# kkty/kmer-sets-compression

Hardware: AMD Instinct MI355X
Metric: Mk-mers/s processed in kmerset-multiple-compress; bytes/k-mer after SPSS (higher is better)
Workload: dtype u32

## Files before the change

include/kmersets_hip.h:

```cpp
#ifndef KMERSETS_HIP_H_
#define KMERSETS_HIP_H_

#include <stddef.h>
#include <stdint.h>

#ifdef __cplusplus
extern "C" {
#endif

#define KSH_OK 0
#define KSH_INVALID_ARGUMENT 3
#define KSH_FAILED_PRECONDITION 9
#define KSH_INTERNAL 13

typedef struct ksh_ctx ksh_ctx;

typedef struct ksh_geom {
  int32_t k;
  int32_t n_bucket_bits;
  int32_t key_bytes;
  int32_t reserved;
} ksh_geom;

typedef struct ksh_set_view {
// ... 105 lines not shown
  KSH_ROUTE_RC_256 = 1 << 3,
  KSH_ROUTE_RC_64 = 1 << 4,
  KSH_ROUTE_RC_BATCHED = 1 << 5,
  KSH_ROUTE_SCATTER_TWO_LEVEL = 1 << 6,
  KSH_ROUTE_FWD_STAGED = 1 << 7,
  KSH_ROUTE_RANK_ONE_LAUNCH = 1 << 8,
  KSH_ROUTE_HEADS_ONE_LAUNCH = 1 << 9,
  KSH_ROUTE_JUMP_TWO_LEVEL = 1 << 10,
  KSH_ROUTE_RANK_STAMPED = 1 << 11,
  KSH_ROUTE_EMIT_LOGS = 1 << 12,
  KSH_ROUTE_LONG_STRETCHES = 1 << 13,
  KSH_ROUTE_MATCH_MORE_ROUNDS = 1 << 14,
  KSH_ROUTE_FWD_TARGETS = 1 << 15,
  KSH_ROUTE_RC1_STREAMED = 1 << 16,
  KSH_ROUTE_RC_MARKS_GROUPS = 1 << 17,
  KSH_ROUTE_TGT_PARTS = 1 << 18
};
int ksh_spss_encode_routes(ksh_ctx* ctx, int64_t* routes);
int ksh_spss_encode_release(ksh_ctx* ctx);

int ksh_spss_cover_plan(ksh_ctx* ctx, const ksh_geom* g, const ksh_spss_view* unitigs, int canonical, int fast,
                        int64_t* n_strings, int64_t* n_bases);
int ksh_spss_cover_write(ksh_ctx* ctx, uint64_t* d_words, uint32_t* d_lens);
int ksh_spss_cover_stats(ksh_ctx* ctx, int64_t stats[4]);
int ksh_spss_cover_release(ksh_ctx* ctx);

typedef struct ksh_kss ksh_kss;
int ksh_kss_build(ksh_ctx* ctx, const ksh_geom* g, const ksh_spss_view* inputs, int32_t n_inputs,
                  const int32_t* bucket_ids, int32_t n_ids, int canonical, int32_t max_iterations,
                  ksh_kss** out);
typedef int (*ksh_allgather_i64)(void* user, const int64_t* send, int64_t count, int64_t* recv);
// ... 66 lines not shown
```

kmer-sets-compression_amd/csrc/ksh_decode.hip:

```cpp
#include "ksh_internal.h"
#include "ksh_kmer.h"

#include <algorithm>
#include <cstdlib>
#include <string>
#include <vector>

namespace ksh {

constexpr int kDecThreads = 1024;
constexpr int kMaxLdsBuckets = 16384;
constexpr int kSortLdsBytes = 63488;
constexpr int kMaxSubBits = 11;
constexpr int kSortThreads = 1024;

__global__ __launch_bounds__(256) void k_str_bases(const uint32_t* __restrict__ lens, int64_t n,
                                                    int k, int64_t* __restrict__ bases) {
  const int64_t i = int64_t(blockIdx.x) * blockDim.x + threadIdx.x;
  if (i < n) bases[i] = int64_t(lens[i]) + k;
}

__global__ __launch_bounds__(256) void k_mark_ends(const int64_t* __restrict__ str_start,
                                                    int64_t n_strings,
                                                    unsigned long long* __restrict__ end_bits) {
  const int64_t i = int64_t(blockIdx.x) * blockDim.x + threadIdx.x;
  if (i >= n_strings) return;
  const int64_t p = str_start[i + 1] - 1;
  atomicOr(&end_bits[p >> 6], 1ull << (p & 63));
}
// ... 236 lines not shown
#pragma unroll
  for (int j = 0; j < kDecL2Per; j++) {
    if (bin[j] == 0xFFFFFFFFu) continue;
    const uint32_t pos = s_lbase[bin[j]] + rank[j];
    s_key[pos] = mine[j];
    s_bin[pos] = uint16_t(bin[j]);
  }
  __syncthreads();
  const uint32_t staged = s_lbase[kBins - 1] + s_cnt[kBins - 1];
  for (uint32_t i = tid; i < staged; i += kDecL2Threads) {
    const uint32_t b = s_bin[i];
    keys[s_gbase[b] + (i - s_lbase[b])] = s_key[i];
  }
}

constexpr int kColTeams = 16;
__global__ __launch_bounds__(64 * kColTeams) void k_hist_columns(uint32_t* __restrict__ hist_matrix,
                                                                  int64_t n_groups, int n_buckets,
                                                                  int64_t* __restrict__ totals,
                                                                  unsigned long long* __restrict__ max_total) {
  __shared__ uint32_t team_total[kColTeams][64];
  const int lane = threadIdx.x & 63, team = threadIdx.x >> 6;
  const int b = blockIdx.x * 64 + lane;
  const int64_t per_team = (n_groups + kColTeams - 1) / kColTeams;
  const int64_t g0 = min(int64_t(team) * per_team, n_groups), g1 = min(g0 + per_team, n_groups);
  uint32_t run = 0;
  if (b < n_buckets)
    for (int64_t g = g0; g < g1; g++) run += hist_matrix[g * n_buckets + b];
  team_total[team][lane] = run;
  __syncthreads();
// ... 24 lines not shown
      if (lane == 0 && max_total) atomicMax(max_total, m);
    } else if (max_total) {
      atomicMax(max_total, m);
    }
  }
}

struct SortLds {
  uint32_t sub_cnt[(1 << kMaxSubBits) + 1];
  int wave_cnt[kSortThreads / 64];
  int wave_below[kSortThreads / 64];
  int overflow;
  int kept;
};

template <typename KeyT>
__device__ void block_sort_into_lds(const KeyT* __restrict__ src, int cnt, int eff_bits,
                                    KeyT* __restrict__ lds, SortLds* __restrict__ sh) {
  int bits = 0;
  while ((4 << bits) < cnt && bits < kMaxSubBits) bits++;
  if (bits > eff_bits) bits = eff_bits;
  const int n_sub = 1 << bits;
  const int shift = eff_bits - bits;
  for (int i = threadIdx.x; i <= n_sub; i += kSortThreads) sh->sub_cnt[i] = 0;
  if (threadIdx.x == 0) sh->overflow = 0;
  constexpr int kSortRegs = 8;
  const bool in_regs = cnt <= kSortRegs * kSortThreads;
  KeyT held[kSortRegs];
  if (in_regs) {
#pragma unroll
    for (int u = 0; u < kSortRegs; u++) {
      const int i = int(threadIdx.x) + u * kSortThreads;
      if (i < cnt) held[u] = src[i];
    }
  }
  __syncthreads();
  if (in_regs) {
#pragma unroll
    for (int u = 0; u < kSortRegs; u++)
      if (int(threadIdx.x) + u * kSortThreads < cnt)
        atomicAdd(&sh->sub_cnt[uint32_t(uint64_t(held[u]) >> shift) & uint32_t(n_sub - 1)], 1u);
  } else {
    for (int i = threadIdx.x; i < cnt; i += kSortThreads)
      atomicAdd(&sh->sub_cnt[uint32_t(uint64_t(src[i]) >> shift) & uint32_t(n_sub - 1)], 1u);
  }
  __syncthreads();
  {
    const int per = (n_sub + kSortThreads - 1) / kSortThreads;
    const int c0 = min(int(threadIdx.x) * per, n_sub), c1 = min(c0 + per, n_sub);
    int mine = 0;
    for (int i = c0; i < c1; i++) mine += int(sh->sub_cnt[i]);
    const int lane = threadIdx.x & 63, wave = threadIdx.x >> 6;
    int inc = mine;
#pragma unroll
    for (int d = 1; d < 64; d <<= 1) {
      const int o = __shfl_up(inc, d, 64);
      if (lane >= d) inc += o;
    }
    if (lane == 63) sh->wave_cnt[wave] = inc;
    __syncthreads();
    int run = inc - mine;
    for (int w = 0; w < wave; w++) run += sh->wave_cnt[w];
    for (int i = c0; i < c1; i++) {
      const int c = int(sh->sub_cnt[i]);
      sh->sub_cnt[i] = uint32_t(run);
      run += c;
    }
  }
  __syncthreads();
  if (in_regs) {
#pragma unroll
    for (int u = 0; u < kSortRegs; u++)
      if (int(threadIdx.x) + u * kSortThreads < cnt) {
        const uint32_t pos = atomicAdd(&sh->sub_cnt[uint32_t(uint64_t(held[u]) >> shift) & uint32_t(n_sub - 1)], 1u);
        lds[pos] = held[u];
      }
  } else {
    for (int i = threadIdx.x; i < cnt; i += kSortThreads) {
      const KeyT key = src[i];
      const uint32_t pos = atomicAdd(&sh->sub_cnt[uint32_t(uint64_t(key) >> shift) & uint32_t(n_sub - 1)], 1u);
      lds[pos] = key;
    }
  }
  __syncthreads();
  for (int b2 = threadIdx.x; b2 < n_sub; b2 += kSortThreads) {
    const int s0 = b2 ? int(sh->sub_cnt[b2 - 1]) : 0, s1 = int(sh->sub_cnt[b2]);
    if (s1 - s0 > 64) {
      sh->overflow = 1;
    } else {
      for (int i = s0 + 1; i < s1; i++) {
        const KeyT x = lds[i];
        int j = i - 1;
        while (j >= s0 && lds[j] > x) {
          lds[j + 1] = lds[j];
          j--;
        }
        lds[j + 1] = x;
      }
    }
  }
  __syncthreads();
  if (sh->overflow == 0) return;
  int padded = 1;
  while (padded < cnt) padded <<= 1;
  const int half = padded >> 1;
  for (int size = 2; size <= padded; size <<= 1) {
    const int hs = size >> 1;
    for (int p = threadIdx.x; p < half; p += kSortThreads) {
      const int block = p / hs, o = p - block * hs;
      const int i = block * size + o, j = block * size + size - 1 - o;
      if (j < cnt) {
        const KeyT x = lds[i], y = lds[j];
        if (x > y) {
          lds[i] = y;
          lds[j] = x;
        }
      }
    }
    __syncthreads();
    for (int stride = size >> 2; stride > 0; stride >>= 1) {
      for (int p = threadIdx.x; p < half; p += kSortThreads) {
        const int i = 2 * stride * (p / stride) + (p % stride), j = i + stride;
        if (j < cnt) {
          const KeyT x = lds[i], y = lds[j];
          if (x > y) {
            lds[i] = y;
            lds[j] = x;
          }
        }
      }
      __syncthreads();
    }
  }
}

template <typename KeyT>
__device__ int block_unique_write(const KeyT* __restrict__ lds, int cnt, KeyT* __restrict__ dst,
                                  SortLds* __restrict__ sh, int cutoff, int64_t* below) {
  const int per = (cnt + kSortThreads - 1) / kSortThreads;
  const int c0 = min(int(threadIdx.x) * per, cnt), c1 = min(c0 + per, cnt);
  int mine = 0, mine_below = 0;
  for (int i = c0; i < c1; i++) {
    if (i == 0 || lds[i] != lds[i - 1]) {
      bool keep = true;
      if (cutoff > 1) {
        int run = 1;
        while (run < cutoff && i + run < cnt && lds[i + run] == lds[i]) run++;
        keep = run >= cutoff;
      }
      mine += keep;
      mine_below += !keep;
    }
  }
  const int lane = threadIdx.x & 63, wave = threadIdx.x >> 6;
// ... 1 lines not shown
#pragma unroll
  for (int d = 1; d < 64; d <<= 1) {
    const int o = __shfl_up(inc, d, 64);
    if (lane >= d) inc += o;
  }
#pragma unroll
  for (int d = 32; d >= 1; d >>= 1) inc_below += __shfl_xor(inc_below, d, 64);
  __syncthreads();
  if (lane == 63) sh->wave_cnt[wave] = inc;
  if (lane == 0) sh->wave_below[wave] = inc_below;
  __syncthreads();
  int at = inc - mine;
  for (int w = 0; w < wave; w++) at += sh->wave_cnt[w];
  int total = 0;
#pragma unroll
  for (int w = 0; w < kSortThreads / 64; w++) total += sh->wave_cnt[w];
  if (threadIdx.x == 0 && below)
    for (int w = 0; w < kSortThreads / 64; w++) *below += sh->wave_below[w];
  if (total == cnt) {
    for (int i = threadIdx.x; i < cnt; i += kSortThreads) dst[i] = lds[i];
    __syncthreads();
    return total;
  }
  for (int i = c0; i < c1; i++) {
    if (i == 0 || lds[i] != lds[i - 1]) {
      bool keep = true;
      if (cutoff > 1) {
        int run = 1;
        while (run < cutoff && i + run < cnt && lds[i + run] == lds[i]) run++;
        keep = run >= cutoff;
      }
      if (keep) dst[at++] = lds[i];
    }
  }
  __syncthreads();
  return total;
}

template <typename KeyT>
__global__ __launch_bounds__(kSortThreads, 8) void k_bucket_sort(const int64_t* __restrict__ offsets,
                                                      KeyT* __restrict__ keys,
                                                      KeyT* __restrict__ scratch,
                                                      int64_t* __restrict__ uniq, int key_bits,
                                                      int cutoff, int64_t* __restrict__ below) {
  extern __shared__ unsigned char lds_raw[];
  __shared__ SortLds sh;
  __shared__ uint32_t part_end[(1 << kMaxSubBits) + 1];
  KeyT* lds = reinterpret_cast<KeyT*>(lds_raw);
  constexpr int kCap = kSortLdsBytes / int(sizeof(KeyT));
  const int64_t b = blockIdx.x;
  const int64_t lo = offsets[b], hi = offsets[b + 1];
  const int64_t cnt64 = hi - lo;
  if (cnt64 == 0) {
    if (threadIdx.x == 0) {
      uniq[b] = 0;
      if (below) below[b] = 0;
    }
    return;
  }
  KeyT* g = keys + lo;
  int64_t n_below = 0;
  if (cnt64 <= kCap) {
    block_sort_into_lds(g, int(cnt64), key_bits, lds, &sh);
    const int kept = block_unique_write(lds, int(cnt64), g, &sh, cutoff, &n_below);
    if (threadIdx.x == 0) {
      uniq[b] = kept;
      if (below) below[b] = n_below;
    }
    return;
  }
  KeyT* tmp = scratch + lo;
  int bits = 1;
  while ((cnt64 >> bits) > kCap / 4 && bits < kMaxSubBits) bits++;
  if (bits > key_bits) bits = key_bits;
  const int n_part = 1 << bits;
  const int shift = key_bits - bits;
  for (int i = threadIdx.x; i <= n_part; i += kSortThreads) part_end[i] = 0;
  __syncthreads();
  for (int64_t i = threadIdx.x; i < cnt64; i += kSortThreads)
    atomicAdd(&part_end[uint32_t(uint64_t(g[i]) >> shift) & uint32_t(n_part - 1)], 1u);
  __syncthreads();
  if (threadIdx.x == 0) {
    uint32_t run = 0;
    for (int i = 0; i < n_part; i++) {
      const uint32_t c = part_end[i];
      part_end[i] = run;
      run += c;
    }
  }
  __syncthreads();
  for (int64_t i = threadIdx.x; i < cnt64; i += kSortThreads) {
    const KeyT key = g[i];
    const uint32_t pos = atomicAdd(&part_end[uint32_t(uint64_t(key) >> shift) & uint32_t(n_part - 1)], 1u);
    tmp[pos] = key;
  }
  __syncthreads();
  int64_t out = 0;
  for (int p = 0; p < n_part; p++) {
    const int64_t s0 = p ? int64_t(part_end[p - 1]) : 0, s1 = int64_t(part_end[p]);
    const int64_t pc = s1 - s0;
    if (pc == 0) continue;
    if (pc <= kCap) {
      block_sort_into_lds(tmp + s0, int(pc), shift, lds, &sh);
      out += block_unique_write(lds, int(pc), g + out, &sh, cutoff, &n_below);
    } else {
      KeyT* buf = tmp + s0;
      int64_t padded = 1;
      while (padded < pc) padded <<= 1;
      const int64_t half = padded >> 1;
      for (int64_t size = 2; size <= padded; size <<= 1) {
        const int64_t hs = size >> 1;
        for (int64_t q = threadIdx.x; q < half; q += kSortThreads) {
          const int64_t block = q / hs, o = q - block * hs;
          const int64_t i = block * size + o, j = block * size + size - 1 - o;
          if (j < pc) {
            const KeyT x = buf[i], y = buf[j];
            if (x > y) {
              buf[i] = y;
              buf[j] = x;
            }
          }
        }
        __syncthreads();
        for (int64_t stride = size >> 2; stride > 0; stride >>= 1) {
          for (int64_t q = threadIdx.x; q < half; q += kSortThreads) {
            const int64_t i = 2 * stride * (q / stride) + (q % stride), j = i + stride;
            if (j < pc) {
              const KeyT x = buf[i], y = buf[j];
              if (x > y) {
                buf[i] = y;
                buf[j] = x;
              }
            }
          }
          __syncthreads();
        }
      }
      if (threadIdx.x == 0) {
        int64_t at = out;
        for (int64_t i = 0; i < pc;) {
// ... 174 lines not shown
  *n_keys = ctx->h_pinned[0];
  ctx->dec_kmers = *n_keys;
  ctx->dec_words = n_words;
  ctx->dec_groups = groups;
  ctx->dec_src = s->d_words;
  return KSH_OK;
}

template <typename KeyT>
int scatter_sort(ksh_ctx* ctx, const ksh_spss_view* s, const DecodeState& st, int k, int nbits_w, int kbw,
                 int canonical_flag, const int64_t* offsets, KeyT* keys, int cutoff, bool want_below,
                 int64_t** new_off, int64_t** below) {
  const int64_t nb = int64_t(1) << nbits_w;
  int64_t n_words, n_end_words, groups, wpg;
  decode_geometry(s, &n_words, &n_end_words, &groups, &wpg);
  static const bool direct = [] {
    const char* e = getenv("KSH_DECODE_SCATTER");
    return e && std::string(e) == "direct";
  }();
  static const int64_t two_level_min = [] {
    const char* e = getenv("KSH_DECODE_L2_MIN");
    return e ? std::max<int64_t>(1024, atoll(e)) : int64_t(1) << 20;
  }();
  if (!direct && ctx->dec_kmers >= two_level_min && nbits_w > kDecSgBits && nbits_w <= 15 &&
      ctx->dec_kmers < int64_t(0xFFFFFFF0)) {
    void* tmp = nullptr;
    const size_t tk = (size_t(ctx->dec_kmers) * sizeof(KeyT) + 255) & ~size_t(255);
    KSH_TRY(pool_alloc(ctx, tk + size_t(ctx->dec_kmers) * 2 + size_t(nb) * 4 + 256, &tmp));
    KeyT* tmp_keys = static_cast<KeyT*>(tmp);
    uint16_t* tmp_b = reinterpret_cast<uint16_t*>(static_cast<char*>(tmp) + tk);
    uint32_t* cursor = reinterpret_cast<uint32_t*>(static_cast<char*>(tmp) + tk + ((size_t(ctx->dec_kmers) * 2 + 255) & ~size_t(255)));
    KSH_HIP(hipMemsetAsync(cursor, 0, size_t(nb) * 4, ctx->stream));
    hipLaunchKernelGGL((k_decode_l1<KeyT>), dim3(unsigned(groups)), dim3(kDecL1Threads), 0, ctx->stream, s->d_words,
                       n_words, s->n_bases, st.end_bits, n_end_words, k, kbw, nbits_w,
                       canonical_flag, wpg, st.hist, offsets, tmp_keys, tmp_b);
    hipLaunchKernelGGL((k_decode_l2<KeyT>), dim3(unsigned((ctx->dec_kmers + kDecL2Tile - 1) / kDecL2Tile)),
                       dim3(kDecL2Threads), 0, ctx->stream, ctx->dec_kmers, nbits_w, offsets, tmp_keys, tmp_b,
                       cursor, keys);
    pool_free(ctx, tmp);
  } else {
    hipLaunchKernelGGL((k_decode<KeyT, true>), dim3(unsigned(groups)), dim3(kDecThreads),
                       size_t(nb) * 4, ctx->stream, s->d_words, n_words, s->n_bases, st.end_bits,
                       n_end_words, k, kbw, int(nb), canonical_flag, wpg, st.hist, offsets,
                       keys);
  }
  KeyT* scratch = nullptr;
  {
    const int64_t max_bucket = ctx->dec_max_bucket;
    if (max_bucket > int64_t(kSortLdsBytes / sizeof(KeyT))) {
      void* ptr = nullptr;
      KSH_TRY(pool_alloc(ctx, size_t(ctx->dec_kmers) * sizeof(KeyT), &ptr));
      scratch = static_cast<KeyT*>(ptr);
    }
  }
  arena_reset(ctx);
  KSH_TRY(arena_reserve(ctx, 2 * a256(size_t(nb + 1) * 8) + (1u << 16)));
  *new_off = static_cast<int64_t*>(arena_alloc(ctx, size_t(nb + 1) * 8));
  *below = static_cast<int64_t*>(arena_alloc(ctx, size_t(nb + 1) * 8));
  if (!*new_off || !*below) return fail(KSH_INTERNAL, "scratch arena too small");
  {
    const uint32_t bit = 8u << (sizeof(KeyT) == 2 ? 0 : sizeof(KeyT) == 4 ? 1 : 2);
    if (!(ctx->lds_opt_in & bit)) {
      KSH_HIP(hipFuncSetAttribute(reinterpret_cast<const void*>(k_bucket_sort<KeyT>),
                                  hipFuncAttributeMaxDynamicSharedMemorySize, kSortLdsBytes));
      ctx->lds_opt_in |= bit;
    }
  }
  hipLaunchKernelGGL((k_bucket_sort<KeyT>), dim3(unsigned(nb)), dim3(kSortThreads), kSortLdsBytes, ctx->stream,
                     offsets, keys, scratch, st.totals, kbw, cutoff, want_below ? *below : nullptr);
  if (scratch) pool_free(ctx, scratch);
  KSH_HIP(hipGetLastError());
  return KSH_OK;
}

template <typename KeyT, typename CT>
int decode_write_wide(ksh_ctx* ctx, const ksh_geom* g, const ksh_spss_view* s, int canonical_flag,
                      int64_t* d_offsets, void* d_keys, int64_t* n_keys, int cutoff, int64_t* n_below) {
  const int64_t nb = n_buckets(g), nbc = int64_t(1) << kCoarseBits;
  const int sub_bits = g->n_bucket_bits - kCoarseBits, cbits = 2 * g->k - kCoarseBits;
  int64_t n_words, n_end_words, groups, wpg;
  decode_geometry(s, &n_words, &n_end_words, &groups, &wpg);
  DecodeState st;
  decode_carve(ctx, groups, nbc, n_end_words, s->n_strings, &st);
  KeyT* keys = static_cast<KeyT*>(d_keys);
// ... 157 lines not shown
```

kmer-sets-compression_amd/csrc/ksh_encode.hip:

```cpp
#include "ksh_internal.h"
#include "ksh_dsu.h"
#include "ksh_kmer.h"

#include <algorithm>
#include <cstddef>
#include <cstdlib>
#include <string>

namespace ksh {

#ifndef KSH_RULER_SHIFT
#define KSH_RULER_SHIFT 5
#endif
constexpr int kRulerShift = KSH_RULER_SHIFT;
constexpr uint32_t kRulerEvery = 1u << kRulerShift;

constexpr uint32_t kNone = 0xFFFFFFFFu;
constexpr uint32_t kMulti = 0xFFFFFFFEu;

#ifndef KSH_JUMP_HOPS
#define KSH_JUMP_HOPS 4
#endif
constexpr int kJumpHops = KSH_JUMP_HOPS;

// ... 225 lines not shown
    const uint64_t rx = revcomp((uint64_t(lo) << set.key_bits) | key, k);
    const uint32_t dst = atomicAdd(&lds_hist[grp], 1u);
    RcRecord<KeyT> r;
    r.key = KeyT(((rx >> (2 * k - 2)) << low_bits) | (rx & low_mask));
    r.t = uint32_t(t);
    rec[dst] = r;
  }
}

constexpr int kSgBits = 7;
constexpr int kL1Threads = 1024;
constexpr int kL2Threads = 256;
constexpr int kL2Per = 8;
constexpr int kL2Tile = kL2Threads * kL2Per;

template <typename KeyT, int kPer>
__global__ __launch_bounds__(kL1Threads) void k_rc_scatter_l1(DevSet<KeyT> set, int nbits, int64_t per_row,
                                                               const uint32_t* __restrict__ hist_matrix,
                                                               const int64_t* __restrict__ goff,
                                                               RcRecord<KeyT>* __restrict__ tmp_rec,
                                                               uint16_t* __restrict__ tmp_g) {
  constexpr int kTile = kL1Threads * kPer;
  constexpr int kSg = 1 << kSgBits;
  __shared__ RcRecord<KeyT> s_rec[kTile];
  __shared__ uint16_t s_g[kTile];
  __shared__ uint32_t s_cur[kSg], s_cnt[kSg], s_lbase[kSg + 1];
  constexpr int kOffCap = 1024;
  __shared__ int64_t s_off[kOffCap];
  const int tid = threadIdx.x;
  const int nb = 1 << nbits, lo_bits = nbits - kSgBits;
  const uint32_t* my_row = hist_matrix + int64_t(blockIdx.x) * nb;
// ... 30 lines not shown
        int l2 = 0, h2 = n_span - 1;
        while (l2 < h2) {
          const int mid = (l2 + h2 + 1) >> 1;
          if (s_off[mid] <= t) l2 = mid; else h2 = mid - 1;
        }
        lo = b_first + l2;
      } else {
        while (lo < hi) {
          const int64_t mid = (lo + hi + 1) >> 1;
          if (set.off[mid] <= t) lo = mid; else hi = mid - 1;
        }
      }
      const uint64_t rx = revcomp((uint64_t(lo) << set.key_bits) | key, k);
      grp[j] = uint32_t(rx >> low_bits) & uint32_t(nb - 1);
      mine[j].key = KeyT(((rx >> (2 * k - 2)) << low_bits) | (rx & low_mask));
      mine[j].t = uint32_t(t);
      rank[j] = atomicAdd(&s_cnt[grp[j] >> lo_bits], 1u);
    }
    __syncthreads();
    if (tid < 64) {
      static_assert(kSg == 128, "two super-groups per lane of one wave");
      const uint32_t c0 = s_cnt[2 * tid], c1 = s_cnt[2 * tid + 1];
      uint32_t inc = c0 + c1;
#pragma unroll
      for (int d = 1; d < 64; d <<= 1) {
        const uint32_t o = __shfl_up(inc, d, 64);
        if (tid >= d) inc += o;
      }
      s_lbase[2 * tid] = inc - c0 - c1;
      s_lbase[2 * tid + 1] = inc - c1;
    }
    __syncthreads();
#pragma unroll
    for (int j = 0; j < kPer; j++) {
      if (grp[j] == 0xFFFFFFFFu) continue;
      const uint32_t pos = s_lbase[grp[j] >> lo_bits] + rank[j];
      s_rec[pos] = mine[j];
      s_g[pos] = uint16_t(grp[j]);
    }
    __syncthreads();
    for (int i = tid; i < tile_n; i += kL1Threads) {
      const uint32_t sg = uint32_t(s_g[i]) >> lo_bits;
      const uint32_t dst = s_cur[sg] + (uint32_t(i) - s_lbase[sg]);
      tmp_rec[dst] = s_rec[i];
      tmp_g[dst] = s_g[i];
    }
    __syncthreads();
    if (tid < kSg) {
      s_cur[tid] += s_cnt[tid];
      s_cnt[tid] = 0;
    }
    __syncthreads();
  }
}

template <typename KeyT>
__global__ __launch_bounds__(kL2Threads) void k_rc_scatter_l2(int64_t n, int nbits, const int64_t* __restrict__ goff,
                                                               const RcRecord<KeyT>* __restrict__ tmp_rec,
                                                               const uint16_t* __restrict__ tmp_g,
                                                               uint32_t* __restrict__ cursor,
// ... 51 lines not shown
  }
  __syncthreads();
#pragma unroll
  for (int j = 0; j < kL2Per; j++) {
    if (bin[j] == 0xFFFFFFFFu) continue;
    const uint32_t pos = s_lbase[bin[j]] + rank[j];
    s_rec[pos] = mine[j];
    s_bin[pos] = uint16_t(bin[j]);
  }
  __syncthreads();
  uint32_t staged = 0;
  for (int b = 0; b < kBins; b++) staged += s_cnt[b];
  for (uint32_t i = tid; i < staged; i += kL2Threads) {
    const uint32_t b = s_bin[i];
    rec[s_gbase[b] + (i - s_lbase[b])] = s_rec[i];
  }
}

template <typename KeyT>
__device__ int64_t lower_bound_kmer(const DevSet<KeyT>& set, uint64_t value) {
  const int64_t b = int64_t(value >> set.key_bits);
  if (b >= set.n_buckets) return set.n;
  const KeyT key = KeyT(value & set.key_mask());
  int64_t lo, hi;
  set.probe_range(b, key, &lo, &hi);
  while (lo < hi) {
    const int64_t mid = (lo + hi) >> 1;
    if (set.keys[mid] < key) lo = mid + 1; else hi = mid;
  }
  return lo;
// ... 2676 lines not shown
  }
  KSH_HIP(hipMemsetAsync(ctl, 0, sizeof(EncCtl) + size_t(2 * nb) * 4, st));
  int* self_rc_flag = &ctl->self_rc;
  {
    Timer timer(ctx, 3, n);
    const int nbits = g->n_bucket_bits;
    if (directed) {
      hipLaunchKernelGGL((k_adjacency<KeyT, true>), dim3(nblk(n)), dim3(256), 0, st, set, p->nbr, self_rc_flag);
    } else if (staged_adjacency() && nbits <= 14 && 2 * g->k >= nbits + 4 &&
               key_bits(g) >= nbits + 2 + (nbits & 1) &&
               n / nb <= 4 * ((kRcWindowBytes - 4 * kRcSegs) / int64_t(sizeof(KeyT) + 6))) {
      const int64_t rows = std::max<int64_t>(1, std::min<int64_t>(kRcRowsMax, (n + 16383) / 16384));
      const int64_t per_row = ((n + rows - 1) / rows + 1023) / 1024 * 1024;
      KSH_BOUND(rows >= 1 && rows <= kRcRowsMax && rows * per_row >= n);
      KSH_BOUND(size_t(n) * sizeof(RcRecord<KeyT>) <= al(size_t(2 * n) * 8));
      static const bool one_level = [] {
        const char* e = getenv("KSH_RC_SCATTER");
        return e && std::string(e) == "direct";
      }();
      static const bool half_groups = [] {
        const char* e = getenv("KSH_RC_GROUPS");
        return e && std::string(e) == "half";
      }();
      const bool two_level = n >= (int64_t(1) << (half_groups ? 12 : 20)) && nbits > kSgBits && nbits <= 16 && !one_level;
      const int extra = (half_groups && two_level && nbits == 14 && key_bits(g) >= 2 * ((nbits + 1 + 2 + 1) / 2)) ? 1 : 0;
      const int gbits = nbits + extra;
      const int64_t ng = int64_t(1) << gbits;
      uint32_t* hist = static_cast<uint32_t*>(arena_alloc(ctx, size_t(rows) * ng * 4));
      int64_t* totals = static_cast<int64_t*>(arena_alloc(ctx, size_t(ng + 1) * 8));
      int64_t* goff = static_cast<int64_t*>(arena_alloc(ctx, size_t(ng + 1) * 8));
      if (!hist || !totals || !goff) return fail(KSH_INTERNAL, "scratch arena too small");
      RcRecord<KeyT>* rec = reinterpret_cast<RcRecord<KeyT>*>(p->info);
      uint32_t* rc0 = p->link;
      uint32_t* rc1 = p->link + n;
// ... 27 lines not shown
      hipLaunchKernelGGL((k_rc_hist<KeyT>), dim3(unsigned(rows)), dim3(1024), hist_lds, st,
                         static_cast<const KeyT*>(sv->d_keys), n, g->k, key_bits(g), gbits, per_row, hist);
      hipLaunchKernelGGL(k_rc_columns, dim3(unsigned((ng + 63) / 64)), dim3(64 * kColTeams), 0, st, hist, rows, int(ng),
                         totals);
      KSH_TRY(scan_exclusive_i64(ctx, totals, goff, ng, goff + ng));
      p->routes |= KSH_ROUTE_PROBE_STAGED | (two_level ? KSH_ROUTE_SCATTER_TWO_LEVEL : 0);
      if (two_level) {
        RcRecord<KeyT>* tmp_rec = sizeof(RcRecord<KeyT>) == 8 ? rec + n : reinterpret_cast<RcRecord<KeyT>*>(p->nbr);
        uint16_t* tmp_g = reinterpret_cast<uint16_t*>(p->head);
        KSH_BOUND(sizeof(RcRecord<KeyT>) == 8 ? size_t(2 * n) * sizeof(RcRecord<KeyT>) <= al(size_t(2 * n) * 8)
                                    : reinterpret_cast<char*>(p->link) == reinterpret_cast<char*>(p->nbr) + al(size_t(2 * n) * 4) &&
                                          size_t(n) * sizeof(RcRecord<KeyT>) <= 2 * al(size_t(2 * n) * 4));
        KSH_BOUND(gbits - kSgBits <= 8);
        uint32_t* cursor = rc_cursor;
        constexpr int kPer = sizeof(RcRecord<KeyT>) == 8 ? 4 : 2;
        hipLaunchKernelGGL((k_rc_scatter_l1<KeyT, kPer>), dim3(unsigned(rows)), dim3(kL1Threads), 0, st, set, gbits,
                           per_row, hist, goff, tmp_rec, tmp_g);
        hipLaunchKernelGGL((k_rc_scatter_l2<KeyT>), dim3(unsigned((n + kL2Tile - 1) / kL2Tile)), dim3(kL2Threads), 0,
                           st, n, gbits, goff, tmp_rec, tmp_g, cursor, rec);
      } else {
        hipLaunchKernelGGL((k_rc_scatter<KeyT>), dim3(unsigned(rows)), dim3(1024), hist_lds, st, set, gbits, 0, 0,
                           per_row, hist, goff, rec);
      }
      const int64_t per_group = n / ng;
      const int cap = int(std::min<int64_t>((kRcWindowBytes - 4 * kRcSegs) / int64_t(sizeof(KeyT) + 6),
                                            std::max<int64_t>(1024, extra ? per_group * 23 / 20 + 256 : per_group * 5 / 4 + 256))) & ~7;
      const size_t rc_lds = size_t(cap) * (sizeof(KeyT) + 4) + size_t(cap + 2 * kRcSegs) * 2;
      KSH_BOUND(cap >= 8 && cap % 8 == 0 && cap + 2 * kRcSegs < 65536);
      KSH_BOUND(rc_lds + 2048 <= size_t(kRcWindowBytes) + 2048 && rc_lds <= size_t(kRcWindowBytes));
      int64_t* pb = static_cast<int64_t*>(arena_alloc(ctx, size_t(ng) * 2 * kRcSegs * 8));
      int64_t* pb0 = extra ? static_cast<int64_t*>(arena_alloc(ctx, size_t(ng) * 2 * 8)) : nullptr;
      if (!pb || (extra && !pb0)) return fail(KSH_INTERNAL, "scratch arena too small");
      hipLaunchKernelGGL((k_rc_bounds<KeyT>), dim3(nblk(ng * 2 * kRcSegs + (extra ? ng * 2 : 0))), dim3(256), 0, st, set,
                         gbits, pb, pb0);
// ... 602 lines not shown
```

kmer-sets-compression_amd/kmersets/capi.py:

```python
import ctypes as C
import os
import subprocess

import numpy as np

PKG_DIR = os.path.dirname(os.path.dirname(os.path.abspath(__file__)))
CSRC_DIR = os.path.join(PKG_DIR, "csrc")
LIB_PATH = os.path.join(CSRC_DIR, "libkmersets_hip.so")
ROOT = os.path.dirname(PKG_DIR)
HEADER = os.path.join(ROOT, "include", "kmersets_hip.h")

KSH_OK, KSH_INVALID_ARGUMENT, KSH_FAILED_PRECONDITION, KSH_INTERNAL = 0, 3, 9, 13


class KshError(RuntimeError):
    def __init__(self, code, message):
        super().__init__("ksh error %d: %s" % (code, message))
        self.code = code


class Geom(C.Structure):
    _fields_ = [("k", C.c_int32), ("n_bucket_bits", C.c_int32), ("key_bytes", C.c_int32),
                ("reserved", C.c_int32)]

# ... 517 lines not shown
        check(lib().ksh_spss_cover_plan(self.h, C.byref(unitigs.g), C.byref(v), int(canonical), int(fast),
                                        C.byref(ns), C.byref(nbases)))
        words = torch.empty(max((nbases.value + 31) // 32, 1), dtype=torch.int64, device=self.device)
        lens = torch.empty(max(ns.value, 1), dtype=torch.int32, device=self.device)
        check(lib().ksh_spss_cover_write(self.h, words.data_ptr(), lens.data_ptr()))
        return DeviceSpss(unitigs.g, words, lens, ns.value, nbases.value)

    def spss_cover_stats(self):
        st = (C.c_int64 * 4)()
        check(lib().ksh_spss_cover_stats(self.h, st))
        return {"unitigs": st[0], "rounds": st[1], "strings": st[2], "bases": st[3]}

    ROUTES = ("probe_staged", "rc_1024", "rc_512", "rc_256", "rc_64", "rc_batched", "scatter_two_level",
              "fwd_staged", "rank_one_launch", "heads_one_launch", "jump_two_level", "rank_stamped", "emit_logs",
              "long_stretches", "match_more_rounds", "fwd_targets", "rc1_streamed", "rc_marks_groups",
              "tgt_parts")

    def spss_encode_routes(self):
        r = C.c_int64()
        check(lib().ksh_spss_encode_routes(self.h, C.byref(r)))
        return {name for bit, name in enumerate(self.ROUTES) if r.value >> bit & 1}

    def pair_algebra_onepass(self, a, b):
        import torch

        g = a.g
        caps = (min(a.n_keys, b.n_keys), a.n_keys, b.n_keys)
        outs = []
        for cap in caps:
            o = DeviceSet.empty_like_offsets(g, 0, self.device)
            o.keys = torch.empty(max(cap * g.key_bytes, 16), dtype=torch.uint8, device=self.device)
# ... 498 lines not shown
```

Before: 27980.

## Share a tiled level-2 scatter, pack bin bits into indices, size bucket-sort LDS

```diff
diff --git a/include/kmersets_hip.h b/include/kmersets_hip.h
--- a/include/kmersets_hip.h
+++ b/include/kmersets_hip.h
@@ -143,7 +143,8 @@
   KSH_ROUTE_FWD_TARGETS = 1 << 15,
   KSH_ROUTE_RC1_STREAMED = 1 << 16,
   KSH_ROUTE_RC_MARKS_GROUPS = 1 << 17,
-  KSH_ROUTE_TGT_PARTS = 1 << 18
+  KSH_ROUTE_TGT_PARTS = 1 << 18,
+  KSH_ROUTE_SCATTER_PACKED = 1 << 19
 };
 int ksh_spss_encode_routes(ksh_ctx* ctx, int64_t* routes);
 int ksh_spss_encode_release(ksh_ctx* ctx);
diff --git a/kmer-sets-compression_amd/csrc/ksh_decode.hip b/kmer-sets-compression_amd/csrc/ksh_decode.hip
--- a/kmer-sets-compression_amd/csrc/ksh_decode.hip
+++ b/kmer-sets-compression_amd/csrc/ksh_decode.hip
@@ -1,5 +1,6 @@
 #include "ksh_internal.h"
 #include "ksh_kmer.h"
+#include "ksh_tile_sort.h"
 
 #include <algorithm>
 #include <cstdlib>
@@ -13,6 +14,9 @@
 constexpr int kSortLdsBytes = 63488;
 constexpr int kMaxSubBits = 11;
 constexpr int kSortThreads = 1024;
+constexpr int kPartEndBytes = ((1 << kMaxSubBits) + 1) * 4;
+constexpr int kSortStaticLds = 8448;
+constexpr int kCuLdsBytes = 160 << 10;
 
 __global__ __launch_bounds__(256) void k_str_bases(const uint32_t* __restrict__ lens, int64_t n,
                                                     int k, int64_t* __restrict__ bases) {
@@ -279,6 +283,19 @@
   }
 }
 
+static_assert(kDecSgBits == kTsSegBits, "level 1 and the shared level 2 cut the bucket at the same bit");
+template <typename KeyT, int kThreads, int kPer>
+__global__ __launch_bounds__(kThreads) void k_decode_l2s(int64_t n, int n_bucket_bits,
+                                                         const int64_t* __restrict__ offsets,
+                                                         const KeyT* __restrict__ tmp_keys,
+                                                         const uint16_t* __restrict__ tmp_b,
+                                                         uint32_t* __restrict__ cursor, KeyT* __restrict__ keys) {
+  const int lo_bits = n_bucket_bits - kDecSgBits;
+  const uint32_t lo_mask = (1u << lo_bits) - 1;
+  tile_sort_l2<KeyT, kThreads, kPer>(
+      n, lo_bits, offsets, tmp_keys, [=](KeyT&, int64_t p) { return uint32_t(tmp_b[p]) & lo_mask; }, cursor, keys);
+}
+
 constexpr int kColTeams = 16;
 __global__ __launch_bounds__(64 * kColTeams) void k_hist_columns(uint32_t* __restrict__ hist_matrix,
                                                                   int64_t n_groups, int n_buckets,
@@ -333,7 +350,7 @@
   int kept;
 };
 
-template <typename KeyT>
+template <typename KeyT, int kT>
 __device__ void block_sort_into_lds(const KeyT* __restrict__ src, int cnt, int eff_bits,
                                     KeyT* __restrict__ lds, SortLds* __restrict__ sh) {
   int bits = 0;
@@ -341,15 +358,15 @@
   if (bits > eff_bits) bits = eff_bits;
   const int n_sub = 1 << bits;
   const int shift = eff_bits - bits;
-  for (int i = threadIdx.x; i <= n_sub; i += kSortThreads) sh->sub_cnt[i] = 0;
+  for (int i = threadIdx.x; i <= n_sub; i += kT) sh->sub_cnt[i] = 0;
   if (threadIdx.x == 0) sh->overflow = 0;
-  constexpr int kSortRegs = 8;
-  const bool in_regs = cnt <= kSortRegs * kSortThreads;
+  constexpr int kSortRegs = 8 * (kSortThreads / kT);
+  const bool in_regs = cnt <= kSortRegs * kT;
   KeyT held[kSortRegs];
   if (in_regs) {
 #pragma unroll
     for (int u = 0; u < kSortRegs; u++) {
-      const int i = int(threadIdx.x) + u * kSortThreads;
+      const int i = int(threadIdx.x) + u * kT;
       if (i < cnt) held[u] = src[i];
     }
   }
@@ -357,15 +374,15 @@
   if (in_regs) {
 #pragma unroll
     for (int u = 0; u < kSortRegs; u++)
-      if (int(threadIdx.x) + u * kSortThreads < cnt)
+      if (int(threadIdx.x) + u * kT < cnt)
         atomicAdd(&sh->sub_cnt[uint32_t(uint64_t(held[u]) >> shift) & uint32_t(n_sub - 1)], 1u);
   } else {
-    for (int i = threadIdx.x; i < cnt; i += kSortThreads)
+    for (int i = threadIdx.x; i < cnt; i += kT)
       atomicAdd(&sh->sub_cnt[uint32_t(uint64_t(src[i]) >> shift) & uint32_t(n_sub - 1)], 1u);
   }
   __syncthreads();
   {
-    const int per = (n_sub + kSortThreads - 1) / kSortThreads;
+    const int per = (n_sub + kT - 1) / kT;
     const int c0 = min(int(threadIdx.x) * per, n_sub), c1 = min(c0 + per, n_sub);
     int mine = 0;
     for (int i = c0; i < c1; i++) mine += int(sh->sub_cnt[i]);
@@ -390,19 +407,19 @@
   if (in_regs) {
 #pragma unroll
     for (int u = 0; u < kSortRegs; u++)
-      if (int(threadIdx.x) + u * kSortThreads < cnt) {
+      if (int(threadIdx.x) + u * kT < cnt) {
         const uint32_t pos = atomicAdd(&sh->sub_cnt[uint32_t(uint64_t(held[u]) >> shift) & uint32_t(n_sub - 1)], 1u);
         lds[pos] = held[u];
       }
   } else {
-    for (int i = threadIdx.x; i < cnt; i += kSortThreads) {
+    for (int i = threadIdx.x; i < cnt; i += kT) {
       const KeyT key = src[i];
       const uint32_t pos = atomicAdd(&sh->sub_cnt[uint32_t(uint64_t(key) >> shift) & uint32_t(n_sub - 1)], 1u);
       lds[pos] = key;
     }
   }
   __syncthreads();
-  for (int b2 = threadIdx.x; b2 < n_sub; b2 += kSortThreads) {
+  for (int b2 = threadIdx.x; b2 < n_sub; b2 += kT) {
     const int s0 = b2 ? int(sh->sub_cnt[b2 - 1]) : 0, s1 = int(sh->sub_cnt[b2]);
     if (s1 - s0 > 64) {
       sh->overflow = 1;
@@ -425,7 +442,7 @@
   const int half = padded >> 1;
   for (int size = 2; size <= padded; size <<= 1) {
     const int hs = size >> 1;
-    for (int p = threadIdx.x; p < half; p += kSortThreads) {
+    for (int p = threadIdx.x; p < half; p += kT) {
       const int block = p / hs, o = p - block * hs;
       const int i = block * size + o, j = block * size + size - 1 - o;
       if (j < cnt) {
@@ -438,7 +455,7 @@
     }
     __syncthreads();
     for (int stride = size >> 2; stride > 0; stride >>= 1) {
-      for (int p = threadIdx.x; p < half; p += kSortThreads) {
+      for (int p = threadIdx.x; p < half; p += kT) {
         const int i = 2 * stride * (p / stride) + (p % stride), j = i + stride;
         if (j < cnt) {
           const KeyT x = lds[i], y = lds[j];
@@ -453,10 +470,10 @@
   }
 }
 
-template <typename KeyT>
+template <typename KeyT, int kT>
 __device__ int block_unique_write(const KeyT* __restrict__ lds, int cnt, KeyT* __restrict__ dst,
                                   SortLds* __restrict__ sh, int cutoff, int64_t* below) {
-  const int per = (cnt + kSortThreads - 1) / kSortThreads;
+  const int per = (cnt + kT - 1) / kT;
   const int c0 = min(int(threadIdx.x) * per, cnt), c1 = min(c0 + per, cnt);
   int mine = 0, mine_below = 0;
   for (int i = c0; i < c1; i++) {
@@ -488,11 +505,11 @@
   for (int w = 0; w < wave; w++) at += sh->wave_cnt[w];
   int total = 0;
 #pragma unroll
-  for (int w = 0; w < kSortThreads / 64; w++) total += sh->wave_cnt[w];
+  for (int w = 0; w < kT / 64; w++) total += sh->wave_cnt[w];
   if (threadIdx.x == 0 && below)
-    for (int w = 0; w < kSortThreads / 64; w++) *below += sh->wave_below[w];
+    for (int w = 0; w < kT / 64; w++) *below += sh->wave_below[w];
   if (total == cnt) {
-    for (int i = threadIdx.x; i < cnt; i += kSortThreads) dst[i] = lds[i];
+    for (int i = threadIdx.x; i < cnt; i += kT) dst[i] = lds[i];
     __syncthreads();
     return total;
   }
@@ -511,17 +528,17 @@
   return total;
 }
 
-template <typename KeyT>
-__global__ __launch_bounds__(kSortThreads, 8) void k_bucket_sort(const int64_t* __restrict__ offsets,
+template <typename KeyT, int kT>
+__global__ __launch_bounds__(kT, kT >= 1024 ? 8 : 6) void k_bucket_sort(const int64_t* __restrict__ offsets,
                                                       KeyT* __restrict__ keys,
                                                       KeyT* __restrict__ scratch,
                                                       int64_t* __restrict__ uniq, int key_bits,
-                                                      int cutoff, int64_t* __restrict__ below) {
+                                                      int cutoff, int64_t* __restrict__ below, int cap) {
   extern __shared__ unsigned char lds_raw[];
   __shared__ SortLds sh;
-  __shared__ uint32_t part_end[(1 << kMaxSubBits) + 1];
   KeyT* lds = reinterpret_cast<KeyT*>(lds_raw);
-  constexpr int kCap = kSortLdsBytes / int(sizeof(KeyT));
+  const int kCap = cap;
+  uint32_t* part_end = reinterpret_cast<uint32_t*>(lds_raw + size_t(cap) * sizeof(KeyT));
   const int64_t b = blockIdx.x;
   const int64_t lo = offsets[b], hi = offsets[b + 1];
   const int64_t cnt64 = hi - lo;
@@ -535,8 +552,8 @@
   KeyT* g = keys + lo;
   int64_t n_below = 0;
   if (cnt64 <= kCap) {
-    block_sort_into_lds(g, int(cnt64), key_bits, lds, &sh);
-    const int kept = block_unique_write(lds, int(cnt64), g, &sh, cutoff, &n_below);
+    block_sort_into_lds<KeyT, kT>(g, int(cnt64), key_bits, lds, &sh);
+    const int kept = block_unique_write<KeyT, kT>(lds, int(cnt64), g, &sh, cutoff, &n_below);
     if (threadIdx.x == 0) {
       uniq[b] = kept;
       if (below) below[b] = n_below;
@@ -549,9 +566,9 @@
   if (bits > key_bits) bits = key_bits;
   const int n_part = 1 << bits;
   const int shift = key_bits - bits;
-  for (int i = threadIdx.x; i <= n_part; i += kSortThreads) part_end[i] = 0;
-  __syncthreads();
-  for (int64_t i = threadIdx.x; i < cnt64; i += kSortThreads)
+  for (int i = threadIdx.x; i <= n_part; i += kT) part_end[i] = 0;
+  __syncthreads();
+  for (int64_t i = threadIdx.x; i < cnt64; i += kT)
     atomicAdd(&part_end[uint32_t(uint64_t(g[i]) >> shift) & uint32_t(n_part - 1)], 1u);
   __syncthreads();
   if (threadIdx.x == 0) {
@@ -563,7 +580,7 @@
     }
   }
   __syncthreads();
-  for (int64_t i = threadIdx.x; i < cnt64; i += kSortThreads) {
+  for (int64_t i = threadIdx.x; i < cnt64; i += kT) {
     const KeyT key = g[i];
     const uint32_t pos = atomicAdd(&part_end[uint32_t(uint64_t(key) >> shift) & uint32_t(n_part - 1)], 1u);
     tmp[pos] = key;
@@ -575,8 +592,8 @@
     const int64_t pc = s1 - s0;
     if (pc == 0) continue;
     if (pc <= kCap) {
-      block_sort_into_lds(tmp + s0, int(pc), shift, lds, &sh);
-      out += block_unique_write(lds, int(pc), g + out, &sh, cutoff, &n_below);
+      block_sort_into_lds<KeyT, kT>(tmp + s0, int(pc), shift, lds, &sh);
+      out += block_unique_write<KeyT, kT>(lds, int(pc), g + out, &sh, cutoff, &n_below);
     } else {
       KeyT* buf = tmp + s0;
       int64_t padded = 1;
@@ -584,7 +601,7 @@
       const int64_t half = padded >> 1;
       for (int64_t size = 2; size <= padded; size <<= 1) {
         const int64_t hs = size >> 1;
-        for (int64_t q = threadIdx.x; q < half; q += kSortThreads) {
+        for (int64_t q = threadIdx.x; q < half; q += kT) {
           const int64_t block = q / hs, o = q - block * hs;
           const int64_t i = block * size + o, j = block * size + size - 1 - o;
           if (j < pc) {
@@ -597,7 +614,7 @@
         }
         __syncthreads();
         for (int64_t stride = size >> 2; stride > 0; stride >>= 1) {
-          for (int64_t q = threadIdx.x; q < half; q += kSortThreads) {
+          for (int64_t q = threadIdx.x; q < half; q += kT) {
             const int64_t i = 2 * stride * (q / stride) + (q % stride), j = i + stride;
             if (j < pc) {
               const KeyT x = buf[i], y = buf[j];
@@ -802,10 +819,12 @@
   const int64_t nb = int64_t(1) << nbits_w;
   int64_t n_words, n_end_words, groups, wpg;
   decode_geometry(s, &n_words, &n_end_words, &groups, &wpg);
-  static const bool direct = [] {
+  static const std::string scatter_env = [] {
     const char* e = getenv("KSH_DECODE_SCATTER");
-    return e && std::string(e) == "direct";
+    return std::string(e ? e : "");
   }();
+  static const bool direct = scatter_env == "direct", r4 = scatter_env == "r4";
+  static const int l2_threads = l2_threads_env(512);
   static const int64_t two_level_min = [] {
     const char* e = getenv("KSH_DECODE_L2_MIN");
     return e ? std::max<int64_t>(1024, atoll(e)) : int64_t(1) << 20;
@@ -822,9 +841,17 @@
     hipLaunchKernelGGL((k_decode_l1<KeyT>), dim3(unsigned(groups)), dim3(kDecL1Threads), 0, ctx->stream, s->d_words,
                        n_words, s->n_bases, st.end_bits, n_end_words, k, kbw, nbits_w,
                        canonical_flag, wpg, st.hist, offsets, tmp_keys, tmp_b);
-    hipLaunchKernelGGL((k_decode_l2<KeyT>), dim3(unsigned((ctx->dec_kmers + kDecL2Tile - 1) / kDecL2Tile)),
-                       dim3(kDecL2Threads), 0, ctx->stream, ctx->dec_kmers, nbits_w, offsets, tmp_keys, tmp_b,
-                       cursor, keys);
+    const int64_t nk = ctx->dec_kmers;
+    constexpr int kP8 = sizeof(KeyT) == 8 ? 4 : 8;
+    auto l2 = [&](auto kernel, int threads, int per) {
+      const int64_t tile = int64_t(threads) * per;
+      hipLaunchKernelGGL(kernel, dim3(unsigned((nk + tile - 1) / tile)), dim3(threads), 0, ctx->stream, nk, nbits_w,
+                         offsets, tmp_keys, tmp_b, cursor, keys);
+    };
+    if (r4) l2(k_decode_l2<KeyT>, kDecL2Threads, kDecL2Per);
+    else if (l2_threads == 256) l2(k_decode_l2s<KeyT, 256, kP8>, 256, kP8);
+    else if (l2_threads == 1024) l2(k_decode_l2s<KeyT, 1024, kP8>, 1024, kP8);
+    else l2(k_decode_l2s<KeyT, 512, kP8>, 512, kP8);
     pool_free(ctx, tmp);
   } else {
     hipLaunchKernelGGL((k_decode<KeyT, true>), dim3(unsigned(groups)), dim3(kDecThreads),
@@ -846,16 +873,35 @@
   *new_off = static_cast<int64_t*>(arena_alloc(ctx, size_t(nb + 1) * 8));
   *below = static_cast<int64_t*>(arena_alloc(ctx, size_t(nb + 1) * 8));
   if (!*new_off || !*below) return fail(KSH_INTERNAL, "scratch arena too small");
+  static const int sort_threads_env = [] {
+    const char* e = getenv("KSH_SORT_THREADS");
+    return e ? atoi(e) : 0;
+  }();
+  const bool oversize = scratch != nullptr;
+  size_t win = kSortLdsBytes;
+  if (!r4 && !oversize)
+    win = std::min<size_t>(kSortLdsBytes, std::max<size_t>(4096, (size_t(ctx->dec_max_bucket) * sizeof(KeyT) + 1023) & ~size_t(1023)));
+  const int cap = int(win / sizeof(KeyT));
+  const size_t sort_lds = win + (oversize ? kPartEndBytes : 0);
+  bool narrow = !r4 && 4 * (sort_lds + kSortStaticLds) <= size_t(kCuLdsBytes);
+  if (!r4 && sort_threads_env == 1024) narrow = false;
+  if (!r4 && sort_threads_env == 512) narrow = true;
   {
     const uint32_t bit = 8u << (sizeof(KeyT) == 2 ? 0 : sizeof(KeyT) == 4 ? 1 : 2);
     if (!(ctx->lds_opt_in & bit)) {
-      KSH_HIP(hipFuncSetAttribute(reinterpret_cast<const void*>(k_bucket_sort<KeyT>),
-                                  hipFuncAttributeMaxDynamicSharedMemorySize, kSortLdsBytes));
+      KSH_HIP(hipFuncSetAttribute(reinterpret_cast<const void*>(k_bucket_sort<KeyT, 1024>),
+                                  hipFuncAttributeMaxDynamicSharedMemorySize, kSortLdsBytes + kPartEndBytes));
+      KSH_HIP(hipFuncSetAttribute(reinterpret_cast<const void*>(k_bucket_sort<KeyT, 512>),
+                                  hipFuncAttributeMaxDynamicSharedMemorySize, kSortLdsBytes + kPartEndBytes));
       ctx->lds_opt_in |= bit;
     }
   }
-  hipLaunchKernelGGL((k_bucket_sort<KeyT>), dim3(unsigned(nb)), dim3(kSortThreads), kSortLdsBytes, ctx->stream,
-                     offsets, keys, scratch, st.totals, kbw, cutoff, want_below ? *below : nullptr);
+  if (narrow)
+    hipLaunchKernelGGL((k_bucket_sort<KeyT, 512>), dim3(unsigned(nb)), dim3(512), sort_lds, ctx->stream, offsets, keys,
+                       scratch, st.totals, kbw, cutoff, want_below ? *below : nullptr, cap);
+  else
+    hipLaunchKernelGGL((k_bucket_sort<KeyT, 1024>), dim3(unsigned(nb)), dim3(1024), sort_lds, ctx->stream, offsets,
+                       keys, scratch, st.totals, kbw, cutoff, want_below ? *below : nullptr, cap);
   if (scratch) pool_free(ctx, scratch);
   KSH_HIP(hipGetLastError());
   return KSH_OK;
diff --git a/kmer-sets-compression_amd/csrc/ksh_encode.hip b/kmer-sets-compression_amd/csrc/ksh_encode.hip
--- a/kmer-sets-compression_amd/csrc/ksh_encode.hip
+++ b/kmer-sets-compression_amd/csrc/ksh_encode.hip
@@ -1,6 +1,7 @@
 #include "ksh_internal.h"
 #include "ksh_dsu.h"
 #include "ksh_kmer.h"
+#include "ksh_tile_sort.h"
 
 #include <algorithm>
 #include <cstddef>
@@ -263,7 +264,7 @@
 constexpr int kL2Per = 8;
 constexpr int kL2Tile = kL2Threads * kL2Per;
 
-template <typename KeyT, int kPer>
+template <typename KeyT, int kPer, bool kPacked = false>
 __global__ __launch_bounds__(kL1Threads) void k_rc_scatter_l1(DevSet<KeyT> set, int nbits, int64_t per_row,
                                                                const uint32_t* __restrict__ hist_matrix,
                                                                const int64_t* __restrict__ goff,
@@ -324,7 +325,7 @@
       const uint64_t rx = revcomp((uint64_t(lo) << set.key_bits) | key, k);
       grp[j] = uint32_t(rx >> low_bits) & uint32_t(nb - 1);
       mine[j].key = KeyT(((rx >> (2 * k - 2)) << low_bits) | (rx & low_mask));
-      mine[j].t = uint32_t(t);
+      mine[j].t = kPacked ? ts_pack(uint32_t(t), grp[j], lo_bits) : uint32_t(t);
       rank[j] = atomicAdd(&s_cnt[grp[j] >> lo_bits], 1u);
     }
     __syncthreads();
@@ -353,7 +354,7 @@
       const uint32_t sg = uint32_t(s_g[i]) >> lo_bits;
       const uint32_t dst = s_cur[sg] + (uint32_t(i) - s_lbase[sg]);
       tmp_rec[dst] = s_rec[i];
-      tmp_g[dst] = s_g[i];
+      if (!kPacked) tmp_g[dst] = s_g[i];
     }
     __syncthreads();
     if (tid < kSg) {
@@ -435,6 +436,31 @@
   for (uint32_t i = tid; i < staged; i += kL2Threads) {
     const uint32_t b = s_bin[i];
     rec[s_gbase[b] + (i - s_lbase[b])] = s_rec[i];
+  }
+}
+
+static_assert(kSgBits == kTsSegBits, "level 1 and the shared level 2 cut the group at the same bit");
+template <typename KeyT, int kThreads, int kPer, bool kPacked>
+__global__ __launch_bounds__(kThreads) void k_rc_scatter_l2s(int64_t n, int nbits, const int64_t* __restrict__ goff,
+                                                             const RcRecord<KeyT>* __restrict__ tmp_rec,
+                                                             const uint16_t* __restrict__ tmp_g,
+                                                             uint32_t* __restrict__ cursor,
+                                                             RcRecord<KeyT>* __restrict__ rec) {
+  const int lo_bits = nbits - kSgBits;
+  if constexpr (kPacked) {
+    tile_sort_l2<RcRecord<KeyT>, kThreads, kPer>(
+        n, lo_bits, goff, tmp_rec,
+        [=](RcRecord<KeyT>& r, int64_t) {
+          const uint32_t low = ts_packed_low(r.t, lo_bits);
+          r.t = ts_packed_index(r.t, lo_bits);
+          return low;
+        },
+        cursor, rec);
+  } else {
+    const uint32_t lo_mask = (1u << lo_bits) - 1;
+    tile_sort_l2<RcRecord<KeyT>, kThreads, kPer>(
+        n, lo_bits, goff, tmp_rec, [=](RcRecord<KeyT>&, int64_t p) { return uint32_t(tmp_g[p]) & lo_mask; }, cursor,
+        rec);
   }
 }
 
@@ -3141,10 +3167,16 @@
       const int64_t per_row = ((n + rows - 1) / rows + 1023) / 1024 * 1024;
       KSH_BOUND(rows >= 1 && rows <= kRcRowsMax && rows * per_row >= n);
       KSH_BOUND(size_t(n) * sizeof(RcRecord<KeyT>) <= al(size_t(2 * n) * 8));
-      static const bool one_level = [] {
+      static const std::string rc_scatter_env = [] {
         const char* e = getenv("KSH_RC_SCATTER");
-        return e && std::string(e) == "direct";
+        return std::string(e ? e : "");
       }();
+      static const bool one_level = rc_scatter_env == "direct", rc_r4 = rc_scatter_env == "r4";
+      static const bool rc_pack = [] {
+        const char* e = getenv("KSH_RC_PACK");
+        return !(e && std::string(e) == "off");
+      }();
+      static const int l2_threads = l2_threads_env(1024);
       static const bool half_groups = [] {
         const char* e = getenv("KSH_RC_GROUPS");
         return e && std::string(e) == "half";
@@ -3202,10 +3234,37 @@
         KSH_BOUND(gbits - kSgBits <= 8);
         uint32_t* cursor = rc_cursor;
         constexpr int kPer = sizeof(RcRecord<KeyT>) == 8 ? 4 : 2;
-        hipLaunchKernelGGL((k_rc_scatter_l1<KeyT, kPer>), dim3(unsigned(rows)), dim3(kL1Threads), 0, st, set, gbits,
-                           per_row, hist, goff, tmp_rec, tmp_g);
-        hipLaunchKernelGGL((k_rc_scatter_l2<KeyT>), dim3(unsigned((n + kL2Tile - 1) / kL2Tile)), dim3(kL2Threads), 0,
-                           st, n, gbits, goff, tmp_rec, tmp_g, cursor, rec);
+        if (rc_r4) {
+          hipLaunchKernelGGL((k_rc_scatter_l1<KeyT, kPer>), dim3(unsigned(rows)), dim3(kL1Threads), 0, st, set, gbits,
+                             per_row, hist, goff, tmp_rec, tmp_g);
+          hipLaunchKernelGGL((k_rc_scatter_l2<KeyT>), dim3(unsigned((n + kL2Tile - 1) / kL2Tile)), dim3(kL2Threads), 0,
+                             st, n, gbits, goff, tmp_rec, tmp_g, cursor, rec);
+        } else {
+          const bool packed = rc_pack && ts_pack_fits(n, gbits - kSgBits);
+          if (packed) p->routes |= KSH_ROUTE_SCATTER_PACKED;
+          if (packed)
+            hipLaunchKernelGGL((k_rc_scatter_l1<KeyT, kPer, true>), dim3(unsigned(rows)), dim3(kL1Threads), 0, st, set,
+                               gbits, per_row, hist, goff, tmp_rec, tmp_g);
+          else
+            hipLaunchKernelGGL((k_rc_scatter_l1<KeyT, kPer>), dim3(unsigned(rows)), dim3(kL1Threads), 0, st, set, gbits,
+                               per_row, hist, goff, tmp_rec, tmp_g);
+          constexpr int kP2 = sizeof(RcRecord<KeyT>) == 8 ? 8 : 4;
+          auto l2 = [&](auto kernel, int threads, int per) {
+            const int64_t tile = int64_t(threads) * per;
+            hipLaunchKernelGGL(kernel, dim3(unsigned((n + tile - 1) / tile)), dim3(threads), 0, st, n, gbits, goff,
+                               tmp_rec, tmp_g, cursor, rec);
+          };
+          if (l2_threads == 256) {
+            if (packed) l2(k_rc_scatter_l2s<KeyT, 256, kP2, true>, 256, kP2);
+            else l2(k_rc_scatter_l2s<KeyT, 256, kP2, false>, 256, kP2);
+          } else if (l2_threads == 1024) {
+            if (packed) l2(k_rc_scatter_l2s<KeyT, 1024, kP2 / 2, true>, 1024, kP2 / 2);
+            else l2(k_rc_scatter_l2s<KeyT, 1024, kP2 / 2, false>, 1024, kP2 / 2);
+          } else {
+            if (packed) l2(k_rc_scatter_l2s<KeyT, 512, kP2, true>, 512, kP2);
+            else l2(k_rc_scatter_l2s<KeyT, 512, kP2, false>, 512, kP2);
+          }
+        }
       } else {
         hipLaunchKernelGGL((k_rc_scatter<KeyT>), dim3(unsigned(rows)), dim3(1024), hist_lds, st, set, gbits, 0, 0,
                            per_row, hist, goff, rec);
diff --git a/kmer-sets-compression_amd/csrc/ksh_tile_sort.h b/kmer-sets-compression_amd/csrc/ksh_tile_sort.h
--- /dev/null
+++ b/kmer-sets-compression_amd/csrc/ksh_tile_sort.h
@@ -0,0 +1,130 @@
+#pragma once
+#include <hip/hip_runtime.h>
+
+#include <cstdint>
+#include <cstdlib>
+
+namespace ksh {
+
+constexpr int kTsSegBits = 7;
+constexpr int kTsSegs = 1 << kTsSegBits;
+constexpr int kTsBins = 512;
+
+__host__ __device__ inline bool ts_pack_fits(int64_t n, int lo_bits) {
+  return lo_bits >= 1 && lo_bits <= 8 && n <= (int64_t(1) << (32 - lo_bits));
+}
+__host__ __device__ inline uint32_t ts_pack(uint32_t index, uint32_t bin, int lo_bits) {
+  return index | ((bin & ((1u << lo_bits) - 1)) << (32 - lo_bits));
+}
+__host__ __device__ inline uint32_t ts_packed_low(uint32_t word, int lo_bits) { return word >> (32 - lo_bits); }
+__host__ __device__ inline uint32_t ts_packed_index(uint32_t word, int lo_bits) {
+  return word & ((1u << (32 - lo_bits)) - 1);
+}
+
+__host__ __device__ inline uint32_t ts_segment_of(const uint32_t* start, uint32_t p) {
+  uint32_t lo = 0, hi = kTsSegs - 1;
+  while (lo < hi) {
+    const uint32_t mid = (lo + hi + 1) >> 1;
+    if (start[mid] <= p) lo = mid; else hi = mid - 1;
+  }
+  return lo;
+}
+
+template <typename Rec, int kThreads, int kPer, typename IdFn>
+__device__ __forceinline__ void tile_sort_l2(int64_t n, int lo_bits, const int64_t* __restrict__ offs,
+                                             const Rec* __restrict__ tmp, IdFn low_id,
+                                             uint32_t* __restrict__ cursor, Rec* __restrict__ out) {
+  static_assert(kThreads >= 256 && kThreads % 64 == 0, "bins are scanned two per thread by the first four waves");
+  constexpr int kTile = kThreads * kPer;
+  __shared__ Rec s_rec[kTile];
+  __shared__ uint16_t s_bin[kTile];
+  __shared__ uint32_t s_cnt[kTsBins], s_lbase[kTsBins], s_gbase[kTsBins];
+  __shared__ uint32_t s_start[kTsSegs + 1];
+  __shared__ uint32_t s_wave[4];
+  const int tid = threadIdx.x;
+  const int64_t p0 = int64_t(blockIdx.x) * kTile;
+  const int tile_n = int(min(int64_t(kTile), n - p0));
+  Rec mine[kPer];
+  uint32_t bin[kPer], rank[kPer];
+#pragma unroll
+  for (int j = 0; j < kPer; j++) {
+    const int i = tid + j * kThreads;
+    bin[j] = 0;
+    if (i < tile_n) {
+      mine[j] = tmp[p0 + i];
+      bin[j] = low_id(mine[j], p0 + i);
+    }
+  }
+  for (int b = tid; b < kTsBins; b += kThreads) s_cnt[b] = 0;
+  if (tid <= kTsSegs) s_start[tid] = uint32_t(offs[int64_t(tid) << lo_bits]);
+  __syncthreads();
+  const uint32_t seg0 = ts_segment_of(s_start, uint32_t(p0));
+  const uint32_t end0 = s_start[seg0 + 1];
+  const uint32_t base = seg0 << lo_bits;
+  const uint32_t n_bins = min(uint32_t(kTsBins), 2u << lo_bits);
+#pragma unroll
+  for (int j = 0; j < kPer; j++) {
+    const int i = tid + j * kThreads;
+    const uint32_t low = bin[j];
+    bin[j] = 0xFFFFFFFFu;
+    if (i >= tile_n) continue;
+    const uint32_t p = uint32_t(p0 + i);
+    const uint32_t seg = p < end0 ? seg0 : ts_segment_of(s_start, p);
+    const uint32_t g = (seg << lo_bits) | low;
+    if (g - base < n_bins) {
+      bin[j] = g - base;
+      rank[j] = atomicAdd(&s_cnt[bin[j]], 1u);
+    } else {
+      out[uint32_t(offs[g]) + atomicAdd(&cursor[g], 1u)] = mine[j];
+    }
+  }
+  __syncthreads();
+  {
+    static_assert(kTsBins == 512, "two bins per thread of four waves");
+    const bool scans = tid < kTsBins / 2;
+    uint32_t c0 = 0, c1 = 0, inc = 0;
+    const int lane = tid & 63, wv = tid >> 6;
+    if (scans) {
+      c0 = s_cnt[2 * tid];
+      c1 = s_cnt[2 * tid + 1];
+      inc = c0 + c1;
+#pragma unroll
+      for (int d = 1; d < 64; d <<= 1) {
+        const uint32_t o = __shfl_up(inc, d, 64);
+        if (lane >= d) inc += o;
+      }
+      if (lane == 63) s_wave[wv] = inc;
+    }
+    __syncthreads();
+    if (scans) {
+      uint32_t before = inc - (c0 + c1);
+      for (int w = 0; w < wv; w++) before += s_wave[w];
+      s_lbase[2 * tid] = before;
+      s_lbase[2 * tid + 1] = before + c0;
+      s_gbase[2 * tid] = c0 ? uint32_t(offs[base + 2 * tid]) + atomicAdd(&cursor[base + 2 * tid], c0) : 0u;
+      s_gbase[2 * tid + 1] = c1 ? uint32_t(offs[base + 2 * tid + 1]) + atomicAdd(&cursor[base + 2 * tid + 1], c1) : 0u;
+    }
+  }
+  __syncthreads();
+#pragma unroll
+  for (int j = 0; j < kPer; j++) {
+    if (bin[j] == 0xFFFFFFFFu) continue;
+    const uint32_t pos = s_lbase[bin[j]] + rank[j];
+    s_rec[pos] = mine[j];
+    s_bin[pos] = uint16_t(bin[j]);
+  }
+  __syncthreads();
+  const uint32_t staged = s_lbase[kTsBins - 1] + s_cnt[kTsBins - 1];
+  for (uint32_t i = tid; i < staged; i += kThreads) {
+    const uint32_t b = s_bin[i];
+    out[s_gbase[b] + (i - s_lbase[b])] = s_rec[i];
+  }
+}
+
+inline int l2_threads_env(int fallback) {
+  const char* e = getenv("KSH_L2_THREADS");
+  const int t = e ? atoi(e) : 0;
+  return t == 256 || t == 512 || t == 1024 ? t : fallback;
+}
+
+}
diff --git a/kmer-sets-compression_amd/kmersets/capi.py b/kmer-sets-compression_amd/kmersets/capi.py
--- a/kmer-sets-compression_amd/kmersets/capi.py
+++ b/kmer-sets-compression_amd/kmersets/capi.py
@@ -555,7 +555,7 @@
     ROUTES = ("probe_staged", "rc_1024", "rc_512", "rc_256", "rc_64", "rc_batched", "scatter_two_level",
               "fwd_staged", "rank_one_launch", "heads_one_launch", "jump_two_level", "rank_stamped", "emit_logs",
               "long_stretches", "match_more_rounds", "fwd_targets", "rc1_streamed", "rc_marks_groups",
-              "tgt_parts")
+              "tgt_parts", "scatter_packed")
 
     def spss_encode_routes(self):
         r = C.c_int64()
```

Result: no change. 28070, median of 3 (+0.3%).
